# SonSang/dmesh_renderer

Hardware: AMD Instinct MI355X
Metric: fwd+bwd Mpixels/sec @1080p, 500k tris; grad max-abs-err vs ref (higher is better)
Workload: dtype f32

## Files before the change

### dmesh_renderer_amd/build.py

```python
from __future__ import annotations

import os
import shutil
import subprocess
import sys

HERE = os.path.dirname(os.path.abspath(__file__))
CSRC = os.path.join(HERE, "csrc")
LIB = os.path.join(HERE, "libdmesh_renderer_hip.so")
LIB_ABLATION = os.path.join(HERE, "libdmesh_renderer_hip_ablation.so")
SOURCES = ["dmr_api.hip", "dmr_binning.hip", "dmr_tri.hip", "dmr_tet.hip", "dmr_shade.hip", "dmr_texture.hip", "dmr_visibility.hip",
           "dmr_interp.hip"]
HEADERS = ["dmr_device.hpp", "dmr_kernels.hpp", "dmr_placement_key.hpp", "dmr_sort.hpp", "dmr_shade_common.hpp", "dmr_texture_wrap.hpp",
           os.path.join("..", "..", "include", "dmesh_renderer_amd.h"), os.path.join("..", "..", "include", "dmesh_renderer_amd_shade.h"),
           os.path.join("..", "..", "include", "dmesh_renderer_amd_texture.h"),
           os.path.join("..", "..", "include", "dmesh_renderer_amd_visibility.h"),
           os.path.join("..", "..", "include", "dmesh_renderer_amd_deferred.h")]
ARCH = "gfx950"


def _hipcc() -> str:
    for cand in (shutil.which("hipcc"), "/opt/rocm/bin/hipcc"):
        if cand and os.path.exists(cand):
            return cand
    raise RuntimeError("hipcc not found: the HIP extension cannot be built")


def _glue_path() -> str:
    import sysconfig
    return os.path.join(HERE, "_C" + (sysconfig.get_config_var("EXT_SUFFIX") or ".so"))


GLUE_SOURCES = ["dmr_torch.cpp", os.path.join("..", "..", "include", "dmesh_renderer_amd.h"),
                os.path.join("..", "..", "include", "dmesh_renderer_amd_shade.h"),
                os.path.join("..", "..", "include", "dmesh_renderer_amd_texture.h"),
                os.path.join("..", "..", "include", "dmesh_renderer_amd_visibility.h"),
                os.path.join("..", "..", "include", "dmesh_renderer_amd_deferred.h")]


def glue_stale() -> bool:
    out = _glue_path()
    if not os.path.exists(out):
        return True
    t = os.path.getmtime(out)
    return any(os.path.getmtime(os.path.join(CSRC, d)) > t for d in GLUE_SOURCES) or os.path.getmtime(os.path.abspath(__file__)) > t


def build_glue(force: bool = False, verbose: bool = False) -> str:
    out = _glue_path()
    if not force and not glue_stale():
        return out
    import sysconfig
    import torch
    from torch.utils import cpp_extension as ce
    tlib = os.path.join(os.path.dirname(torch.__file__), "lib")
    cxx = shutil.which("g++") or shutil.which("c++")
    if not cxx:
        raise RuntimeError("g++ not found: the PyTorch binding cannot be built")
    cmd = [cxx, "-O2", "-std=c++17", "-fPIC", "-shared", "-D__HIP_PLATFORM_AMD__=1", "-DUSE_ROCM=1", "-DTORCH_EXTENSION_NAME=_C",
           "-DTORCH_API_INCLUDE_EXTENSION_H", f"-D_GLIBCXX_USE_CXX11_ABI={int(torch._C._GLIBCXX_USE_CXX11_ABI)}"]
    cmd += ["-I" + p for p in ce.include_paths()] + ["-I/opt/rocm/include", "-I" + sysconfig.get_paths()["include"]]
    cmd += [os.path.join(CSRC, "dmr_torch.cpp"), "-o", out + ".tmp", "-L" + tlib, "-lc10", "-lc10_hip", "-ltorch_cpu", "-ltorch_hip",
            "-ltorch", "-ltorch_python", "-Wl,-rpath," + tlib, "-ldl"]
    if verbose:
        print(" ".join(cmd), flush=True)
    subprocess.check_call(cmd)
    os.replace(out + ".tmp", out)
    return out


def build_all(force: bool = False, verbose: bool = False):
    res = build(force=force, verbose=verbose), build_glue(force=force, verbose=verbose)
    pkg = sys.modules.get(__package__ or "dmesh_renderer_amd")
    if pkg is not None and type(getattr(pkg, "_C", None)).__name__ == "_NotBuilt":
        import importlib
        pkg._C = importlib.import_module(pkg.__name__ + "._C")
    return res


def stale(lib: str = LIB) -> bool:
    if not os.path.exists(lib):
        return True
    t = os.path.getmtime(lib)
    deps = [os.path.join(CSRC, s) for s in SOURCES + HEADERS] + [os.path.abspath(__file__)]
    return any(os.path.getmtime(d) > t for d in deps)


def build(force: bool = False, verbose: bool = False, ablation: bool = False) -> str:
    lib = LIB_ABLATION if ablation else LIB
    if not force and not stale(lib):
        return lib
    cmd = [_hipcc(), f"--offload-arch={ARCH}", "-O3", "-std=c++17", "-ffp-contract=off", "-fno-slp-vectorize", "-fPIC", "-shared",
           "-Wall", "-Wno-unused-function", "-Wl,-rpath,/opt/rocm/lib", "-o", lib + ".tmp"]
    if ablation:
        cmd.append("-DDMR_ABLATION")
    cmd += [os.path.join(CSRC, s) for s in SOURCES]
    if verbose:
        print(" ".join(cmd), flush=True)
    subprocess.check_call(cmd)
    os.replace(lib + ".tmp", lib)
    return lib


if __name__ == "__main__":
    print(build(force="--force" in sys.argv, verbose=True, ablation="--ablation" in sys.argv))
    if "--ablation" not in sys.argv:
        print(build_glue(force="--force" in sys.argv, verbose=True))
```

### dmesh_renderer_amd/csrc/dmr_api.hip

```cpp
#include <algorithm>
#include <atomic>
#include <chrono>
#include <cstdio>
#include <cstdlib>
#include <cstring>
#include <functional>
#include <map>
#include <mutex>
#include <string>
#include <vector>

#include "dmr_kernels.hpp"
#include "dmr_placement_key.hpp"

namespace {

thread_local std::string g_err;

int fail(const std::string& m) { g_err = m; return 1; }

#define DMR_HIP(expr)                                                                           \
    do {                                                                                        \
        hipError_t e_ = (expr);                                                                 \
        if (e_ != hipSuccess) return fail(std::string(#expr) + ": " + hipGetErrorString(e_));   \
    } while (0)

int caller_output(dmr_alloc_fn alloc, void* ctx, int which, size_t bytes, const char* what, bool idle, hipStream_t st, float** out) {
    *out = nullptr;
    if (bytes == 0) return 0;
    if (!alloc) return fail("null argument");
    float* p = static_cast<float*>(alloc(ctx, which, bytes));
    if (!p) return fail(std::string("allocation of the ") + what + " buffer failed");
    if (idle) DMR_HIP(hipMemsetAsync(p, 0, bytes, st));
    else *out = p;
    return 0;
}

int fragment_k(const dmr_scene* s, int flag, const char* name, const char* macro) {
    const int K = (s->flags & flag) ? DMR_FRAGMENTS_K(s->flags) : 0;
    if ((s->flags & flag) && (K < 1 || K > dmr::FRAG_MAX_K))
        return -fail(std::string(name) + ": K (bits 8-15 of flags, " + macro + ") must be in 1..32, got " + std::to_string(K));
    return K;
}

int fragment_grad_inputs(dmr_alloc_fn alloc, void* ctx, const char* r, const std::string& R, int face_id, int grad_id, size_t npix, int K,
                         const int32_t** face, const float** grad) {
    if (!alloc) return fail("null argument");
    const std::string no = "DMR_FLAG_" + R + "_FRAGMENT_GRADS: no " + r + " fragment ";
    *face = static_cast<const int32_t*>(alloc(ctx, face_id, dmr::FragmentLists::face_bytes(npix, K)));
    if (!*face) return fail(no + "face buffer (DMR_BUF_" + R + "_FRAGMENT_FACES)");
    *grad = static_cast<const float*>(alloc(ctx, grad_id, dmr::FragmentLists::bary_bytes(npix, K)));
    if (!*grad) return fail(no + "bary gradient buffer (DMR_BUF_" + R + "_FRAGMENT_BARY_GRADS)");
    return 0;
}

using dmr::Dims;
using dmr::PointState;
using dmr::FaceState;
using dmr::ImageState;
using dmr::BinningState;
using dmr::Scratch;

constexpr size_t ALIGN = 256;
inline size_t up(size_t n) { return (n + ALIGN - 1) & ~(ALIGN - 1); }

struct Carver {
    char* base; size_t off;
    explicit Carver(void* b) : base(reinterpret_cast<char*>(b)), off(0) {}
    template <class T> T* take(size_t count) {
        T* p = base ? reinterpret_cast<T*>(base + off) : nullptr;
        off += up(count * sizeof(T));
        return p;
    }
};

size_t carve_point(void* b, size_t BP, PointState& s) { Carver c(b); s.vproj = c.take<float4>(BP); return c.off; }
size_t carve_face(void* b, size_t BF, size_t F, size_t T, bool tet, FaceState& s) {
    Carver c(b);
    s.rect = c.take<uint2>(BF); s.key_depth = c.take<float>(BF);
    s.max_depth = tet ? c.take<float>(BF) : nullptr;
    s.tiles_touched = c.take<uint32_t>(BF);
    s.facerec = s.colrec = s.tetrec = nullptr;
    if (tet) {
        s.facerec = c.take<char>(F * dmr::tet_facerec_bytes());
        s.colrec = c.take<char>(F * dmr::tet_colrec_bytes());
        s.tetrec = c.take<char>(T * dmr::tet_tetrec_bytes());
    }
    return c.off;
}
size_t carve_image(void* b, size_t B, size_t ntiles, size_t npix, bool tet, ImageState& s) {
    Carver c(b);
    s.mats = c.take<float>(64 * B);
    s.seed = c.take<int>(1);
    s.mask_offset = c.take<unsigned long long>(2);
    s.tile_count = c.take<uint32_t>(ntiles); s.tile_hits = c.take<uint32_t>(ntiles); s.tile_bound = c.take<uint32_t>(ntiles);
    s.scan_tmp = c.take<uint32_t>(dmr::scan_tmp_words((int)ntiles));
    s.hit_offset = c.take<uint32_t>(ntiles + 1); s.tile_used = c.take<uint32_t>(ntiles); s.hit_total = c.take<unsigned long long>(1);
    s.tile_offset = c.take<uint32_t>(ntiles + 1);
    s.tile_cursor = c.take<uint32_t>(ntiles); s.num_rendered = c.take<int>(1);
    s.tile_order = c.take<uint32_t>(ntiles);
    s.final_T = c.take<float>(npix); s.final_prev_T = c.take<float>(npix); s.n_contrib = c.take<uint32_t>(npix);
    if (tet) {
        s.first_face = c.take<int32_t>(npix); s.first_tet = c.take<int32_t>(npix);
        s.last_face = c.take<int32_t>(npix); s.last_tet = c.take<int32_t>(npix);
        s.is_active = c.take<uint8_t>(npix);
        s.seq = c.take<dmr::TetSeq>(1);
    } else {
        s.first_face = s.first_tet = s.last_face = s.last_tet = nullptr; s.is_active = nullptr;
        s.seq = nullptr;
    }
    return c.off;
}
size_t carve_binning(void* b, size_t R, size_t mask_tiles, size_t seq_tiles, size_t seq_steps, BinningState& s) {
    Carver c(b);
    s.face_list = c.take<uint32_t>(R); s.keys = c.take<uint64_t>(R);
    s.capacity = (uint32_t)std::min<size_t>(R, 0xffffffffu);
    s.mask_offset = c.off;
    s.mask_first = dmr::mask_first_slots(R, mask_tiles);
    if (mask_tiles && R > 0) c.take<uint4>(dmr::mask_slots(R, mask_tiles) * 256);
    s.base = reinterpret_cast<char*>(b); s.seq_offset = c.off; s.seq_steps = (uint32_t)seq_steps;
    if (seq_steps) c.take<char>(dmr::tet_seq_bytes(seq_tiles, seq_steps));
    return c.off;
}

Scratch carve_scratch(const dmr_scene* s, bool tet, const Dims& d, const void* pb, const void* fb, const void* ib,
                      const void* bb = nullptr, size_t R = 0) {
    Scratch c;
    c.point_bytes = carve_point(const_cast<void*>(pb), d.BP, c.ps);
    c.face_bytes = carve_face(const_cast<void*>(fb), d.BF, (size_t)s->F, (size_t)s->T, tet, c.fs);
    c.image_bytes = carve_image(const_cast<void*>(ib), (size_t)s->B, (size_t)d.ntiles, d.npix, tet, c.is);
    carve_binning(const_cast<void*>(bb), R, 0, 0, 0, c.bs);
    return c;
}
dmr_scene canonical(const dmr_scene* s, const float* mats) {
    dmr_scene c = *s;
    const size_t n = 16 * (size_t)s->B;
    c.mv_mats = mats; c.proj_mats = mats + n; c.inv_mv_mats = mats + 2 * n; c.inv_proj_mats = mats + 3 * n;
    c.mats_transposed = 0;
    return c;
}

int check_scene(const dmr_scene* s, bool tet, Dims& d) {
    if (!s) return fail("null scene");
    if (s->B <= 0 || s->W <= 0 || s->H <= 0 || s->P < 0 || s->F < 0 || s->T < 0) return fail("bad dimensions");
    if ((int64_t)s->B * s->P > INT32_MAX || (int64_t)s->B * s->F > INT32_MAX || (int64_t)s->B * s->W * s->H > INT32_MAX)
        return fail("problem too large for 32-bit indexing");
    d.gx = (s->W + dmr::TILE - 1) / dmr::TILE;
    d.gy = (s->H + dmr::TILE - 1) / dmr::TILE;
    if (d.gx > 65535 || d.gy > 65535) return fail("image too large (tile coordinates must fit 16 bits)");
    d.r0 = s->row_begin; d.r1 = s->row_end;
    if (d.r0 == 0 && d.r1 == 0) d.r1 = d.gy;
    d.r0 = std::max(0, std::min(d.gy, d.r0));
    d.r1 = std::max(d.r0, std::min(d.gy, d.r1));
    d.ntiles = s->B * d.gx * d.gy;
    d.BP = (size_t)s->B * s->P; d.BF = (size_t)s->B * s->F; d.npix = (size_t)s->B * s->W * s->H;
    if (tet && s->F > 0 && s->P > 0 && (!s->tets || !s->face_tets || !s->tet_faces)) return fail("tet topology missing");
    if (tet && s->F >= (1 << 28)) return fail("too many faces for the tet renderer (face ids must fit 28 bits)");
    return 0;
}

void* pinned_words() {
    void* p = nullptr;
    if (hipHostMalloc(&p, 64, hipHostMallocCoherent | hipHostMallocPortable) != hipSuccess) return nullptr;
    memset(p, 0, 64);
    return p;
}

struct SizeRead {
    void* slot = nullptr; uint32_t seq = 0;
    volatile unsigned long long* word(int which) const { return reinterpret_cast<volatile unsigned long long*>(slot) + which; }
    uint32_t next_seq() { seq = (seq + 1u) & 0xffffffu; if (seq == 0u) seq = 1u; return seq; }
};
thread_local std::map<int, SizeRead> g_size_read;
int wait_size(volatile unsigned long long* w, uint32_t seq, hipStream_t st, unsigned long long* size) {
    const auto t0 = std::chrono::steady_clock::now();
    for (uint32_t spins = 0;; spins++) {
        const unsigned long long v = *w;
        if ((uint32_t)(v >> 40) == (seq & 0xffffffu)) { std::atomic_thread_fence(std::memory_order_acquire); *size = v & ((1ull << 40) - 1ull); return 0; }
        if ((spins & 1023u) == 1023u && std::chrono::steady_clock::now() - t0 > std::chrono::milliseconds(50)) break;
#if defined(__x86_64__) || defined(__i386__)
        __builtin_ia32_pause();
#endif
    }
    DMR_HIP(hipStreamSynchronize(st));
    const unsigned long long v = *w;
    if ((uint32_t)(v >> 40) != (seq & 0xffffffu)) return fail("the size word was not written (internal error)");
    *size = v & ((1ull << 40) - 1ull);
    return 0;
}

std::mutex g_overflow_mu;
std::map<int, uint32_t*> g_overflow;
uint32_t* overflow_word(int dev, bool create) {
    std::lock_guard<std::mutex> lk(g_overflow_mu);
    auto it = g_overflow.find(dev);
    if (it != g_overflow.end()) return it->second;
    if (!create) return nullptr;
    void* p = pinned_words();
    if (!p) return nullptr;
    return g_overflow[dev] = reinterpret_cast<uint32_t*>(p);
}

bool is_async(const dmr_scene* s, hipStream_t st) {
    if (s->flags & DMR_FLAG_ASYNC) return true;
    hipStreamCaptureStatus cs = hipStreamCaptureStatusNone;
    if (hipStreamIsCapturing(st, &cs) != hipSuccess) { (void)hipGetLastError(); return false; }
    return cs != hipStreamCaptureStatusNone;
}

struct SizeKey {
    int v[7];
    bool operator<(const SizeKey& o) const { return memcmp(v, o.v, sizeof(v)) < 0; }
};
struct SizeGuess { double rendered_per_face = 0.0, hits_per_face = 0.0; uint32_t* seq_steps = nullptr; };
std::mutex g_size_mu;
std::map<SizeKey, SizeGuess> g_size_cache;
std::atomic<uint64_t> g_redo_count{0};
int size_bucket(size_t BF) { int b = 0; while ((BF >> (b + 1)) != 0) b++; return b; }
SizeKey size_key(const dmr_scene* s, bool tet, const Dims& d) {
    return SizeKey{{s->B, s->W, s->H, d.r0, d.r1, tet ? 1 : 0, size_bucket(d.BF)}};
}
double lookup_estimate(const SizeKey& key, double SizeGuess::* field) {
    for (int db : {0, -1, 1}) {
        SizeKey k = key; k.v[6] += db;
        auto it = g_size_cache.find(k);
        if (it != g_size_cache.end() && it->second.*field > 0.0) return it->second.*field;
    }
    return 0.0;
}
uint64_t padded(uint64_t n) { return n + n / 4 + 4096; }

struct Placement { uint32_t* start = nullptr; uint32_t* order = nullptr; int ntiles = 0; uint64_t capacity = 0, built_from = 0; bool valid = false; };
std::mutex g_placement_mu;
std::map<dmr::PlacementKey, Placement> g_placement;
int current_device() { int dev = 0; if (hipGetDevice(&dev) != hipSuccess) { (void)hipGetLastError(); dev = -1; } return dev; }
dmr::PlacementKey placement_key(const SizeKey& key) { return dmr::placement_key(current_device(), key.v, 7); }
uint64_t placement_capacity(uint64_t R, int ntiles) { return R + R / 4 + (uint64_t)dmr::SEG_SLACK * (uint64_t)ntiles; }
bool placement_eligible(bool tet, const Dims& d) { return !tet && d.ntiles <= dmr::SCAN_SINGLE_MAX; }
Placement find_placement(const SizeKey& key, const Dims& d) {
    const dmr::PlacementKey pk = placement_key(key);
    if (pk.device < 0) return Placement{};
    std::lock_guard<std::mutex> lk(g_size_mu);
    auto it = g_placement.find(pk);
    return it != g_placement.end() && it->second.valid && it->second.ntiles == d.ntiles ? it->second : Placement{};
}
void drop_placement(const SizeKey& key) {
    const dmr::PlacementKey pk = placement_key(key);
    std::lock_guard<std::mutex> lk(g_size_mu);
    auto it = g_placement.find(pk);
    if (it != g_placement.end()) it->second.valid = false;
}
int build_placement(const SizeKey& key, const Dims& d, uint64_t R, const ImageState& is, hipStream_t st) {
    const uint64_t capacity = placement_capacity(R, d.ntiles);
    if (capacity > 0x7fffffffu) { drop_placement(key); return 0; }
    const dmr::PlacementKey pk = placement_key(key);
    if (pk.device < 0) return 0;
    std::lock_guard<std::mutex> build_lk(g_placement_mu);
    Placement p;
    {
        std::lock_guard<std::mutex> lk(g_size_mu);
        p = g_placement[pk];
        g_placement[pk].valid = false;
    }
    if (p.start && p.ntiles != d.ntiles) return 0;
    if (!p.start) {
        void* mem = nullptr;
        DMR_HIP(hipMalloc(&mem, sizeof(uint32_t) * (2 * (size_t)d.ntiles + 1)));
        p.start = reinterpret_cast<uint32_t*>(mem); p.order = p.start + d.ntiles + 1; p.ntiles = d.ntiles;
    } else {
        DMR_HIP(hipDeviceSynchronize());
    }
    dmr::launch_build_placement(d.ntiles, is.tile_count, is.tile_order, p.start, p.order, st);
    DMR_HIP(hipStreamSynchronize(st));
    p.capacity = capacity; p.built_from = R; p.valid = true;
    std::lock_guard<std::mutex> lk(g_size_mu);
    g_placement[pk] = p;
    return 0;
}

constexpr uint64_t TET_SEQ_BUDGET = 16ull << 30;
uint64_t march_budget_steps(const Dims& d) {
    return std::max<uint64_t>(TET_SEQ_BUDGET / std::max<uint64_t>(dmr::tet_seq_bytes((size_t)d.ntiles, 4), 1), 1) * 4;
}
uint32_t* march_estimate(const SizeKey& key, const Dims& d, bool create, size_t* seq_steps = nullptr) {
    std::lock_guard<std::mutex> lk(g_size_mu);
    SizeGuess& g = g_size_cache[key];
    if (!g.seq_steps && create && !(g.seq_steps = reinterpret_cast<uint32_t*>(pinned_words()))) (void)hipGetLastError();
    if (seq_steps) {
        const uint64_t longest = g.seq_steps ? *reinterpret_cast<volatile uint32_t*>(g.seq_steps) : 0u;
        *seq_steps = longest ? (size_t)std::min<uint64_t>((longest + longest / 4 + 4 + 3) / 4 * 4, march_budget_steps(d)) : 0;
    }
    return g.seq_steps;
}

using dmr::SizeOut;
using dmr::NOWHERE;

struct Sizing { double SizeGuess::* estimate; uint64_t limit; int word; const char* too_large; const char* no_estimate; };

template <class First, class Then>
int sized(const Sizing& z, const SizeKey& key, size_t BF, bool async, hipStream_t st, uint64_t placed_capacity, uint64_t* size, First first, Then then) {
    int dev = 0;
    DMR_HIP(hipGetDevice(&dev));
    uint32_t* overflow = overflow_word(dev, !async);
    uint64_t guess = placed_capacity;
    if (!placed_capacity) {
        std::lock_guard<std::mutex> lk(g_size_mu);
        const double per_face = lookup_estimate(key, z.estimate);
        if (per_face > 0.0) guess = std::min<uint64_t>(padded((uint64_t)(per_face * (double)BF)), z.limit);
    }
    if (async) {
        if (!guess || !overflow) return fail(z.no_estimate);
        if (first(guess, SizeOut{nullptr, overflow, 0u, (uint32_t)guess})) return 1;
        *size = guess;
        DMR_HIP(hipGetLastError());
        return 0;
    }
    SizeRead& sr = g_size_read[dev];
    if (!sr.slot && !(sr.slot = pinned_words())) return fail("hipHostMalloc failed");
    const uint32_t seq = sr.next_seq();
    if (first(guess, SizeOut{const_cast<unsigned long long*>(sr.word(z.word)), nullptr, seq, 0xffffffffu})) return 1;
    unsigned long long n = 0;
    if (wait_size(sr.word(z.word), seq, st, &n)) return 1;
    const bool full = placed_capacity ? (n & dmr::SIZE_WORD_OVERFLOW) != 0 : n > guess;
    if (placed_capacity) n &= dmr::SIZE_WORD_OVERFLOW - 1ull;
    if (n > z.limit) return fail(z.too_large);
    *size = n;
    if (!guess) {
        if (then(n, false)) return 1;
    } else if (full) {
        g_redo_count.fetch_add(1, std::memory_order_relaxed);
        DMR_HIP(hipStreamSynchronize(st));
        if (then(n, true)) return 1;
    }
    {
        std::lock_guard<std::mutex> lk(g_size_mu);
        g_size_cache[key].*z.estimate = (double)std::max<uint64_t>(n, 1) / (double)std::max<size_t>(BF, 1);
    }
    DMR_HIP(hipGetLastError());
    return 0;
}

int run_forward(const dmr_scene* s, bool tet, const Dims& d, dmr_alloc_fn alloc, void* ctx, hipStream_t st, int* num_rendered,
                const std::function<void(const Scratch&, dmr::ListSize)>& render, size_t min_seq_steps = 0) {
    const Scratch need = carve_scratch(s, tet, d, nullptr, nullptr, nullptr);
    void* pb = alloc(ctx, DMR_BUF_POINT, need.point_bytes);
    void* fb = alloc(ctx, DMR_BUF_FACE, need.face_bytes);
    void* ib = alloc(ctx, DMR_BUF_IMAGE, need.image_bytes);
    if (!pb || !fb || !ib) return fail("scratch allocation failed");
    Scratch c = carve_scratch(s, tet, d, pb, fb, ib);
    const bool async = is_async(s, st);
    const SizeKey key = size_key(s, tet, d);
    size_t seq_steps = 0;
    if (tet) march_estimate(key, d, !async, &seq_steps);
    seq_steps = std::max(seq_steps, min_seq_steps);
    const bool placed = placement_eligible(tet, d);
    const Placement pl = placed ? find_placement(key, d) : Placement{};

    auto front = [&](SizeOut out) {
        dmr::launch_project_verts(*s, d, c, dmr::NO_SEGMENTS, st);
        dmr::launch_setup_faces(*s, d, c, tet, st);
        dmr::launch_scan_tiles(d, c, out, st);
    };
    auto binning = [&](uint64_t capacity) -> int {
        BinningState tb;
        const size_t mask_tiles = tet ? 0 : (size_t)d.ntiles;
        void* bb = alloc(ctx, DMR_BUF_BINNING, carve_binning(nullptr, (size_t)capacity, mask_tiles, (size_t)d.ntiles, seq_steps, tb));
        if (!bb && (capacity > 0 || seq_steps > 0)) return fail("binning allocation failed");
        carve_binning(bb, (size_t)capacity, mask_tiles, (size_t)d.ntiles, seq_steps, c.bs);
        return 0;
    };
    bool exact = false;
    auto rest = [&](uint64_t capacity) -> int {
        if (binning(capacity)) return 1;
        exact = true;
        if (capacity > 0) {
            dmr::launch_scatter_faces(*s, d, c, !tet, st);
            if (!dmr::sorts_own_tiles(d)) dmr::launch_sort_tiles(d, c, st);
        }
        render(c, dmr::NO_LIST_SIZE);
        return 0;
    };
    auto binned = [&](SizeOut out) -> int {
        if (binning(pl.capacity)) return 1;
        dmr::launch_project_verts(*s, d, c, dmr::SegInit{pl.start, pl.order}, st);
        dmr::launch_bin_faces(*s, d, c, st);
        render(c, dmr::ListSize{c.is.num_rendered, out, 1u});
        return 0;
    };

    const Sizing list_entries{&SizeGuess::rendered_per_face, 0x7fffffffu, 0, "num_rendered overflows 31 bits",
                              "asynchronous / captured call without a size estimate: run one default (waiting) call with the same "
                              "view configuration first"};
    uint64_t R = 0;
    int rc = sized(list_entries, key, d.BF, async, st, pl.valid ? pl.capacity : 0, &R,
                   [&](uint64_t guess, SizeOut out) {
                       if (pl.valid) return binned(out);
                       front(out);
                       return guess ? rest(guess) : 0;
                   },
                   [&](uint64_t size, bool redo) { if (redo) front(NOWHERE); return rest(size); });
    *num_rendered = (int)R;
    if (rc == 0 && placed && !async) {
        if (exact) rc = build_placement(key, d, R, c.is, st);
        else if (2 * R < pl.built_from) drop_placement(key);
    }
    return rc;
}

std::atomic<uint32_t> g_prof_mask{0};
struct ProfRec { int stage; hipEvent_t a, b; };
std::mutex g_prof_mu;
std::vector<ProfRec*> g_prof_live, g_prof_free;

}

namespace dmr {
StageScope::StageScope(int stage_, hipStream_t st_) : stage(stage_), st(st_), rec(nullptr) {
    if (!(g_prof_mask.load(std::memory_order_relaxed) & (1u << stage))) return;
    ProfRec* r = nullptr;
    {
        std::lock_guard<std::mutex> lk(g_prof_mu);
        if (!g_prof_free.empty()) { r = g_prof_free.back(); g_prof_free.pop_back(); }
    }
    if (!r) {
        r = new ProfRec();
        if (hipEventCreate(&r->a) != hipSuccess || hipEventCreate(&r->b) != hipSuccess) { delete r; return; }
    }
    r->stage = stage;
    (void)hipEventRecord(r->a, st);
    rec = r;
}
StageScope::~StageScope() {
    if (!rec) return;
    ProfRec* r = reinterpret_cast<ProfRec*>(rec);
    (void)hipEventRecord(r->b, st);
    std::lock_guard<std::mutex> lk(g_prof_mu);
    g_prof_live.push_back(r);
}
int api_fail(const char* m) { return fail(m); }
}

extern "C" {

void dmr_profile_enable(uint32_t mask) { g_prof_mask.store(mask); }

int dmr_profile_collect(double* ms, int64_t* launches) {
    std::vector<ProfRec*> live;
    {
        std::lock_guard<std::mutex> lk(g_prof_mu);
        live.swap(g_prof_live);
    }
    int rc = 0;
    for (ProfRec* r : live) {
        float t = 0.f;
        if (hipEventSynchronize(r->b) != hipSuccess || hipEventElapsedTime(&t, r->a, r->b) != hipSuccess) {
            g_err = "profile event read failed";
            rc = 1;
        } else if (r->stage >= 0 && r->stage < DMR_NUM_STAGES) {
            if (ms) ms[r->stage] += (double)t;
            if (launches) launches[r->stage] += 1;
        }
    }
    std::lock_guard<std::mutex> lk(g_prof_mu);
    for (ProfRec* r : live) g_prof_free.push_back(r);
    return rc;
}

const char* dmr_stage_name(int stage) {
    static const char* names[DMR_NUM_STAGES] = {"k_project_verts", "k_setup_faces", "k_scan_tiles", "k_scatter_faces",
                                                "k_sort_tiles", "k_tri_forward", "k_tri_backward_pix", "k_tri_unpack",
                                                "k_tet_first_intersect", "k_tet_forward", "k_tet_backward",
                                                "k_tri_backward_hits"};
    return (stage >= 0 && stage < DMR_NUM_STAGES) ? names[stage] : "?";
}

const char* dmr_last_error(void) { return g_err.c_str(); }

int dmr_overflowed(int device, int reset) {
    int dev = device;
    if (dev < 0 && hipGetDevice(&dev) != hipSuccess) return 0;
    uint32_t* w = overflow_word(dev, false);
    if (!w) return 0;
    volatile uint32_t* v = w;
    const int r = *v != 0u;
    if (reset) *v = 0u;
    return r;
}
uint64_t dmr_redo_count(void) { return g_redo_count.load(std::memory_order_relaxed); }
int dmr_abi_version(void) { return DMR_ABI_VERSION; }
const char* dmr_build_arch(void) { return "gfx950"; }

int dmr_tri_forward(const dmr_scene* s, float* out_color, float* out_depth, dmr_alloc_fn alloc, void* ctx,
                    void* stream, int* num_rendered) {
    Dims d;
    if (check_scene(s, false, d)) return 1;
    if (!alloc || !num_rendered || !out_color || !out_depth) return fail("null argument");
    *num_rendered = 0;
    const int frag_k = fragment_k(s, DMR_FLAG_TRI_FRAGMENTS, "DMR_FLAG_TRI_FRAGMENTS", "DMR_FRAGMENTS_FLAGS(K)");
    if (frag_k < 0) return 1;
    if (s->P == 0 || s->F == 0) return 0;
    hipStream_t st = reinterpret_cast<hipStream_t>(stream);
    float* fragments = nullptr;
    if (caller_output(alloc, ctx, DMR_BUF_TRI_FRAGMENTS, frag_k ? dmr::FragmentLists::bytes(d.npix, frag_k) : 0, "tri fragment", false, st, &fragments))
        return 1;
    Scratch last{};
    auto render = [&](const Scratch& c, dmr::ListSize size) {
        dmr::launch_tri_forward(canonical(s, c.is.mats), d, c, out_color, out_depth, (s->flags & DMR_FLAG_ALPHA) != 0, size, st);
        last = c;
    };
    if (run_forward(s, false, d, alloc, ctx, st, num_rendered, render)) return 1;
    if (fragments && last.is.n_contrib) {
        dmr::launch_tri_fragments(canonical(s, last.is.mats), d, last, frag_k, fragments, st);
        DMR_HIP(hipGetLastError());
    }
    return 0;
}

int dmr_tri_backward(const dmr_scene* s, const float* dL_dcolor, const float* dL_ddepth, int num_rendered,
                     const void* point_buf, const void* face_buf, const void* binning_buf, const void* image_buf,
                     float* dL_dverts, float* dL_dvcolor, float* dL_dfopacity, float* dL_dvdepth, float* dL_dfintense,
                     dmr_alloc_fn alloc, void* ctx, void* stream) {
    Dims d;
    if (check_scene(s, false, d)) return 1;
    hipStream_t st = reinterpret_cast<hipStream_t>(stream);
    const int frag_k = fragment_k(s, DMR_FLAG_TRI_FRAGMENT_GRADS, "DMR_FLAG_TRI_FRAGMENT_GRADS", "DMR_FRAGMENTS_K");
    if (frag_k < 0) return 1;
    const bool camera = (s->flags & DMR_FLAG_TRI_CAMERA_GRADS) != 0;
    const int grads = camera ? dmr::TRI_GRAD_CAMERA : ((s->flags & DMR_FLAG_TRI_EXACT_GRADS) ? dmr::TRI_GRAD_EXACT : dmr::TRI_GRAD_REF);
    const bool idle = s->P == 0 || s->F == 0 || num_rendered <= 0 || d.r1 <= d.r0;
    float* cam_out = nullptr;
    if (caller_output(alloc, ctx, DMR_BUF_TRI_CAMERA_GRADS, camera ? 128 * (size_t)s->B : 0, "tri camera gradient", idle, st, &cam_out)) return 1;
    const int32_t* frag_face = nullptr;
    const float* frag_grad = nullptr;
    if (frag_k && !idle && fragment_grad_inputs(alloc, ctx, "tri", "TRI", DMR_BUF_TRI_FRAGMENT_FACES, DMR_BUF_TRI_FRAGMENT_BARY_GRADS, d.npix, frag_k, &frag_face, &frag_grad))
        return 1;
    if (idle) {
        if (s->P > 0) {
            DMR_HIP(hipMemsetAsync(dL_dverts, 0, sizeof(float) * 3 * (size_t)s->P, st));
            DMR_HIP(hipMemsetAsync(dL_dvcolor, 0, sizeof(float) * 3 * (size_t)s->P, st));
            DMR_HIP(hipMemsetAsync(dL_dvdepth, 0, sizeof(float) * d.BP, st));
        }
        if (s->F > 0) {
            DMR_HIP(hipMemsetAsync(dL_dfopacity, 0, sizeof(float) * (size_t)s->F, st));
            DMR_HIP(hipMemsetAsync(dL_dfintense, 0, sizeof(float) * d.BF, st));
        }
        if (s->P > 0 && s->F > 0) {
            std::lock_guard<std::mutex> lk(g_size_mu);
            SizeGuess& g = g_size_cache[size_key(s, false, d)];
            if (!(g.hits_per_face > 0.0)) g.hits_per_face = 1.0 / (double)std::max<size_t>(d.BF, 1);
        }
        return 0;
    }
    if (!point_buf || !face_buf || !binning_buf || !image_buf || !alloc) return fail("null scratch buffer");
    const Scratch c = carve_scratch(s, false, d, point_buf, face_buf, image_buf, binning_buf, (size_t)num_rendered);
    const ImageState& is = c.is;

    const size_t vbytes = up(sizeof(float) * dmr::VROW * d.BP), fbytes = up(sizeof(float) * dmr::FROW * d.BF);
    const size_t pbytes = up(sizeof(float4) * 2 * (size_t)d.ntiles * dmr::TILE_PIX);
    const size_t cbytes = camera ? up(sizeof(float) * 32 * (size_t)d.ntiles) : 0;
    auto rest = [&](uint64_t capacity, dmr::HitRegions regions) -> int {
        const size_t hbytes = up(sizeof(dmr::HitRecord) * (size_t)capacity);
        char* work = reinterpret_cast<char*>(alloc(ctx, DMR_BUF_WORK, vbytes + fbytes + cbytes + pbytes + hbytes));
        if (!work) return fail("workspace allocation failed");
        float* vrow = reinterpret_cast<float*>(work);
        float* frow = reinterpret_cast<float*>(work + vbytes);
        float* cam_part = reinterpret_cast<float*>(work + vbytes + fbytes);
        float4* pixrec = reinterpret_cast<float4*>(work + vbytes + fbytes + cbytes);
        dmr::HitRecord* hits = reinterpret_cast<dmr::HitRecord*>(work + vbytes + fbytes + cbytes + pbytes);
        const dmr_scene sc = canonical(s, is.mats);
        dmr::launch_tri_backward_pix(sc, d, c, dL_dcolor, dL_ddepth, pixrec, hits, (uint32_t)capacity, reinterpret_cast<float*>(work),
                                     (vbytes + fbytes + cbytes) / sizeof(float), regions,
                                     (s->flags & DMR_FLAG_ALPHA) != 0, st);
        dmr::launch_tri_backward_hits(sc, d, c, pixrec, hits, (uint32_t)capacity, vrow, frow, grads, camera ? cam_part : nullptr, st);
        if (frag_face)
            dmr::launch_tri_fragment_grads(sc, d, c, frag_k, frag_face, frag_grad, vrow, camera ? cam_part : nullptr, st);
        dmr::launch_tri_unpack(*s, vrow, frow, dL_dverts, dL_dvcolor, dL_dfopacity, dL_dvdepth, dL_dfintense, st);
        if (camera) dmr::launch_camera_reduce(s->B, d.gx * d.gy, 32, cam_part, cam_out, st);
        return 0;
    };
    const dmr::HitRegions scanned{nullptr, nullptr, NOWHERE};
    auto self_laid = [&](SizeOut out) { return dmr::HitRegions{is.hit_offset, is.hit_total, out}; };
    const bool self_regions = d.ntiles <= dmr::SCAN_SINGLE_MAX;
    auto first = [&](uint64_t guess, SizeOut out) -> int {
        if (guess && self_regions) return rest(guess, self_laid(out));
        dmr::launch_scan_hits(d, c, out, st);
        return guess ? rest(guess, scanned) : 0;
    };
    const Sizing hit_records{&SizeGuess::hits_per_face, 0xfffffffeu, 1, "more than 2^32 blended (pixel, face) pairs",
                             "asynchronous / captured call without a size estimate: run one default (waiting) backward with the "
                             "same view configuration first"};
    uint64_t nhits = 0;
    return sized(hit_records, size_key(s, false, d), d.BF, is_async(s, st), st, 0, &nhits, first,
                 [&](uint64_t exact, bool redo) { return rest(exact, redo && self_regions ? self_laid(NOWHERE) : scanned); });
}

int dmr_tet_forward(const dmr_scene* s, float* out_color, float* out_depth, float* out_active, dmr_alloc_fn alloc,
                    void* ctx, void* stream, int* num_rendered) {
    Dims d;
    if (check_scene(s, true, d)) return 1;
    if (!alloc || !num_rendered || !out_color || !out_depth || !out_active) return fail("null argument");
    *num_rendered = 0;
    hipStream_t st = reinterpret_cast<hipStream_t>(stream);
    int frag_k = fragment_k(s, DMR_FLAG_TET_FRAGMENTS, "DMR_FLAG_TET_FRAGMENTS", "DMR_TET_FRAGMENTS_FLAGS(K)");
    if (frag_k < 0) return 1;
    if (s->P == 0 || s->F == 0) frag_k = 0;
    const size_t frag_steps = ((size_t)frag_k + 3) / 4 * 4;
    if (frag_steps > march_budget_steps(d))
        return fail("DMR_FLAG_TET_FRAGMENTS: K = " + std::to_string(frag_k) + " needs a march sequence of " +
                    std::to_string(dmr::tet_seq_bytes((size_t)d.ntiles, frag_steps)) + " bytes (" + std::to_string(frag_steps) +
                    " steps for each of " + std::to_string((size_t)d.ntiles * dmr::TILE_PIX) + " tile pixels), beyond the budget of " +
                    std::to_string(TET_SEQ_BUDGET) + " bytes (16 GiB)");
    float* fragments = nullptr;
    if (caller_output(alloc, ctx, DMR_BUF_TET_FRAGMENTS, frag_k ? dmr::FragmentLists::bytes(d.npix, frag_k) : 0, "tet fragment", false, st, &fragments))
        return 1;
    auto render = [&](const Scratch& c, dmr::ListSize) {
        const dmr_scene sc = canonical(s, c.is.mats);
        dmr::launch_tet_prep(sc, d, c, st);
        dmr::launch_tet_first_intersect(sc, d, c, st);
        dmr::launch_tet_forward(sc, d, c, out_color, out_depth, out_active, (s->flags & DMR_FLAG_ALPHA) != 0, st);
        if (fragments) dmr::launch_tet_fragments(sc, d, c, frag_k, fragments, st);
    };
    return run_forward(s, true, d, alloc, ctx, st, num_rendered, render, frag_steps);
}

int dmr_tet_backward(const dmr_scene* s, const float* dL_dcolor, const float* dL_ddepth, const void* point_buf,
                     const void* face_buf, const void* binning_buf, const void* image_buf, float* dL_dvcolor,
                     float* dL_dfopacity, dmr_alloc_fn alloc, void* ctx, void* stream) {
    Dims d;
    if (check_scene(s, true, d)) return 1;
    hipStream_t st = reinterpret_cast<hipStream_t>(stream);
    const int frag_k = fragment_k(s, DMR_FLAG_TET_FRAGMENT_GRADS, "DMR_FLAG_TET_FRAGMENT_GRADS", "DMR_FRAGMENTS_K");
    if (frag_k < 0) return 1;
    const bool camera = (s->flags & DMR_FLAG_TET_CAMERA_GRADS) != 0;
    const int band_tiles = d.gx * (d.r1 - d.r0);
    float* cam_out = nullptr;
    if (caller_output(alloc, ctx, DMR_BUF_TET_CAMERA_GRADS, camera ? 256 * (size_t)s->B : 0, "tet camera gradient",
                      s->P == 0 || s->F == 0 || band_tiles == 0, st, &cam_out))
        return 1;
    float* full = nullptr;
    const bool full_grads = (s->flags & (DMR_FLAG_TET_FULL_GRADS | DMR_FLAG_TET_CAMERA_GRADS | DMR_FLAG_TET_FRAGMENT_GRADS)) != 0;
    if (caller_output(alloc, ctx, DMR_BUF_TET_GRADS, full_grads ? sizeof(float) * (3 * (size_t)s->P + d.BF) : 0, "tet gradient", false, st, &full))
        return 1;
    if (full) dmr::launch_tet_zero_grads(full, 3 * (int64_t)s->P, full + 3 * (int64_t)s->P, (int64_t)d.BF, st);
    dmr::launch_tet_zero_grads(dL_dvcolor, 3 * (int64_t)s->P, dL_dfopacity, (int64_t)s->F, st);
    if (s->P == 0 || s->F == 0) return 0;
    if (!image_buf || !face_buf) return fail("null scratch buffer");
    const int32_t* frag_face = nullptr;
    const float* frag_grad = nullptr;
    if (frag_k && band_tiles > 0 && fragment_grad_inputs(alloc, ctx, "tet", "TET", DMR_BUF_TET_FRAGMENT_FACES, DMR_BUF_TET_FRAGMENT_BARY_GRADS, d.npix, frag_k, &frag_face, &frag_grad))
        return 1;
    float* cam_part = nullptr;
    if (cam_out) {
        cam_part = static_cast<float*>(alloc(ctx, DMR_BUF_WORK, 256 * (size_t)band_tiles * (size_t)s->B));
        if (!cam_part) return fail("workspace allocation failed");
    }
    const Scratch c = carve_scratch(s, true, d, point_buf, face_buf, image_buf, binning_buf);
    const dmr_scene sc = canonical(s, c.is.mats);
    uint32_t* host_seq_steps = march_estimate(size_key(s, true, d), d, false);
    dmr::launch_tet_backward(sc, d, c, dL_dcolor, dL_ddepth, dL_dvcolor, dL_dfopacity, host_seq_steps, full,
                             full ? full + 3 * (int64_t)s->P : nullptr, cam_part, (s->flags & DMR_FLAG_ALPHA) != 0, st);
    if (frag_face) dmr::launch_tet_fragment_grads(sc, d, c, frag_k, frag_face, frag_grad, full, cam_part, st);
    if (cam_out) dmr::launch_camera_reduce(s->B, band_tiles, 64, cam_part, cam_out, st);
    DMR_HIP(hipGetLastError());
    return 0;
}

namespace {
__global__ void k_invert_mats(const float* __restrict__ in, int count, int transposed, float* __restrict__ out) {
    const int m = blockIdx.x * blockDim.x + threadIdx.x;
    if (m >= count) return;
    double a[16];
#pragma unroll
    for (int k = 0; k < 16; k++) a[k] = (double)in[16 * m + (transposed ? 4 * (k & 3) + (k >> 2) : k)];
    const double s0 = a[0] * a[5] - a[1] * a[4], s1 = a[0] * a[6] - a[2] * a[4], s2 = a[0] * a[7] - a[3] * a[4];
    const double s3 = a[1] * a[6] - a[2] * a[5], s4 = a[1] * a[7] - a[3] * a[5], s5 = a[2] * a[7] - a[3] * a[6];
    const double c5 = a[10] * a[15] - a[11] * a[14], c4 = a[9] * a[15] - a[11] * a[13], c3 = a[9] * a[14] - a[10] * a[13];
    const double c2 = a[8] * a[15] - a[11] * a[12], c1 = a[8] * a[14] - a[10] * a[12], c0 = a[8] * a[13] - a[9] * a[12];
    const double det = s0 * c5 - s1 * c4 + s2 * c3 + s3 * c2 - s4 * c1 + s5 * c0;
    const double r = 1.0 / det;
    double b[16];
    b[0] = (a[5] * c5 - a[6] * c4 + a[7] * c3) * r;   b[1] = (-a[1] * c5 + a[2] * c4 - a[3] * c3) * r;
    b[2] = (a[13] * s5 - a[14] * s4 + a[15] * s3) * r; b[3] = (-a[9] * s5 + a[10] * s4 - a[11] * s3) * r;
    b[4] = (-a[4] * c5 + a[6] * c2 - a[7] * c1) * r;  b[5] = (a[0] * c5 - a[2] * c2 + a[3] * c1) * r;
    b[6] = (-a[12] * s5 + a[14] * s2 - a[15] * s1) * r; b[7] = (a[8] * s5 - a[10] * s2 + a[11] * s1) * r;
    b[8] = (a[4] * c4 - a[5] * c2 + a[7] * c0) * r;   b[9] = (-a[0] * c4 + a[1] * c2 - a[3] * c0) * r;
    b[10] = (a[12] * s4 - a[13] * s2 + a[15] * s0) * r; b[11] = (-a[8] * s4 + a[9] * s2 - a[11] * s0) * r;
    b[12] = (-a[4] * c3 + a[5] * c1 - a[6] * c0) * r; b[13] = (a[0] * c3 - a[1] * c1 + a[2] * c0) * r;
    b[14] = (-a[12] * s3 + a[13] * s1 - a[14] * s0) * r; b[15] = (a[8] * s3 - a[9] * s1 + a[10] * s0) * r;
#pragma unroll
    for (int k = 0; k < 16; k++) out[16 * m + k] = (float)b[k];
}
}

int dmr_invert_mats(const float* in, int count, int transposed, float* out, void* stream) {
    if (count < 0 || (count > 0 && (!in || !out))) return fail("dmr_invert_mats: bad arguments");
    if (count == 0) return 0;
    hipStream_t st = reinterpret_cast<hipStream_t>(stream);
    k_invert_mats<<<dim3((unsigned)((count + 63) / 64)), dim3(64), 0, st>>>(in, count, transposed, out);
    DMR_HIP(hipGetLastError());
    return 0;
}

namespace {
__global__ void k_export_vproj(const float4* v, int64_t n, int what, float* dst) {
    const int64_t i = (int64_t)blockIdx.x * blockDim.x + threadIdx.x;
    if (i >= n) return;
    if (what == 0) { dst[2 * i] = v[i].x; dst[2 * i + 1] = v[i].y; }
    else dst[i] = v[i].z;
}
__global__ void k_export_ranges(const uint32_t* off, const uint32_t* cnt, int64_t n, uint32_t* dst) {
    const int64_t i = (int64_t)blockIdx.x * blockDim.x + threadIdx.x;
    if (i >= n) return;
    const bool empty = cnt[i] == 0;
    dst[2 * i] = empty ? 0u : off[i];
    dst[2 * i + 1] = empty ? 0u : off[i + 1];
}
}

int64_t dmr_export(const dmr_scene* s, int is_tet, int num_rendered, const char* name, const void* point_buf,
                   const void* face_buf, const void* binning_buf, const void* image_buf, void* dst, int64_t cap,
                   void* stream) {
    Dims d;
    if (!name || check_scene(s, is_tet != 0, d)) return -1;
    hipStream_t st = reinterpret_cast<hipStream_t>(stream);
    const Scratch c = carve_scratch(s, is_tet != 0, d, point_buf, face_buf, image_buf, binning_buf, (size_t)std::max(0, num_rendered));
    const FaceState& fs = c.fs; const ImageState& is = c.is;
    const std::string n(name);
    auto plain = [&](const void* src, size_t bytes) -> int64_t {
        if (dst && src && bytes) {
            if (hipMemcpyAsync(dst, src, std::min<size_t>(bytes, (size_t)cap), hipMemcpyDeviceToDevice, st) != hipSuccess) {
                g_err = "export copy failed";
                return -1;
            }
        }
        return (int64_t)bytes;
    };
    if (n == "image" || n == "ndc_z") {
        const size_t bytes = d.BP * (n == "image" ? 8 : 4);
        if (dst && d.BP && (size_t)cap >= bytes)
            k_export_vproj<<<dim3((unsigned)((d.BP + 255) / 256)), dim3(256), 0, st>>>(
                c.ps.vproj, (int64_t)d.BP, n == "image" ? 0 : 1, reinterpret_cast<float*>(dst));
        return (int64_t)bytes;
    }
    if (!is_tet && d.ntiles <= dmr::SCAN_SINGLE_MAX && (n == "ranges" || n == "face_list")) {
        const size_t nt = (size_t)d.ntiles, R = (size_t)std::max(0, num_rendered);
        const size_t bytes = n == "ranges" ? nt * 8 : R * 4;
        if (!dst || (size_t)cap < bytes || bytes == 0) return (int64_t)bytes;
        if (!image_buf || (n == "face_list" && !binning_buf)) { g_err = "null scratch buffer"; return -1; }
        std::vector<uint32_t> off(nt + 1), end(nt), out(bytes / 4, 0u);
        if (hipStreamSynchronize(st) != hipSuccess || hipMemcpy(off.data(), is.tile_offset, 4 * (nt + 1), hipMemcpyDeviceToHost) != hipSuccess ||
            hipMemcpy(end.data(), is.tile_cursor, 4 * nt, hipMemcpyDeviceToHost) != hipSuccess) { g_err = "export copy failed"; return -1; }
        std::vector<uint32_t> lists;
        if (n == "face_list") {
            lists.resize(off[nt]);
            if (off[nt] && hipMemcpy(lists.data(), c.bs.face_list, 4 * (size_t)off[nt], hipMemcpyDeviceToHost) != hipSuccess) { g_err = "export copy failed"; return -1; }
        }
        size_t run = 0;
        for (size_t t = 0; t < nt; t++) {
            const size_t len = dmr::list_end(off.data(), end.data(), (int)t) - off[t];
            if (n == "ranges") { out[2 * t] = len ? (uint32_t)run : 0u; out[2 * t + 1] = len ? (uint32_t)(run + len) : 0u; }
            else for (size_t k = 0; k < len && run + k < R; k++) out[run + k] = lists[off[t] + k];
            run += len;
        }
        if (hipMemcpy(dst, out.data(), bytes, hipMemcpyHostToDevice) != hipSuccess) { g_err = "export copy failed"; return -1; }
        return (int64_t)bytes;
    }
    if (n == "ranges") {
        const size_t bytes = (size_t)d.ntiles * 8;
        if (dst && (size_t)cap >= bytes)
            k_export_ranges<<<dim3((unsigned)((d.ntiles + 255) / 256)), dim3(256), 0, st>>>(
                is.tile_offset, is.tile_count, d.ntiles, reinterpret_cast<uint32_t*>(dst));
        return (int64_t)bytes;
    }
    if (n == "key_depth") return plain(fs.key_depth, d.BF * 4);
    if (n == "max_depth") return is_tet ? plain(fs.max_depth, d.BF * 4) : -1;
    if (n == "tiles_touched") return plain(fs.tiles_touched, d.BF * 4);
    if (n == "face_list") return plain(c.bs.face_list, (size_t)std::max(0, num_rendered) * 4);
    if (n == "final_T") return plain(is.final_T, d.npix * 4);
    if (n == "final_prev_T") return plain(is.final_prev_T, d.npix * 4);
    if (n == "n_contrib") return plain(is.n_contrib, d.npix * 4);
    if (n == "tile_hits") return is_tet ? -1 : plain(is.tile_hits, (size_t)d.ntiles * 4);
    if (is_tet) {
        if (n == "first_face") return plain(is.first_face, d.npix * 4);
        if (n == "first_tet") return plain(is.first_tet, d.npix * 4);
        if (n == "last_face") return plain(is.last_face, d.npix * 4);
        if (n == "last_tet") return plain(is.last_tet, d.npix * 4);
        if (n == "is_active") return plain(is.is_active, d.npix);
        if (n == "tet_seq") return plain(is.seq, 8);
    }
    g_err = "unknown export item: " + n;
    return -1;
}

}
```

Measured before the change: 7805.

## Reorder tile dispatch with host-side block-aware load balancing across XCD classes

After building placement, tile counts and hit counts are copied to the host. A greedy partitioner there assigns 4x4 tile blocks to 8 interleaved classes, which likely correspond to the XCDs, balancing estimated cost. Within each class tiles are sorted longest-first, and the resulting order overwrites the device-built order. The aim is to keep spatially adjacent tiles on the same die for cache locality and to balance per-die work. The cost is host round-trips and synchronisation on the placement build path.

```diff
diff --git a/dmesh_renderer_amd/build.py b/dmesh_renderer_amd/build.py
--- a/dmesh_renderer_amd/build.py
+++ b/dmesh_renderer_amd/build.py
@@ -11,7 +11,7 @@
 LIB_ABLATION = os.path.join(HERE, "libdmesh_renderer_hip_ablation.so")
 SOURCES = ["dmr_api.hip", "dmr_binning.hip", "dmr_tri.hip", "dmr_tet.hip", "dmr_shade.hip", "dmr_texture.hip", "dmr_visibility.hip",
            "dmr_interp.hip"]
-HEADERS = ["dmr_device.hpp", "dmr_kernels.hpp", "dmr_placement_key.hpp", "dmr_sort.hpp", "dmr_shade_common.hpp", "dmr_texture_wrap.hpp",
+HEADERS = ["dmr_device.hpp", "dmr_kernels.hpp", "dmr_placement_key.hpp", "dmr_tile_order.hpp", "dmr_sort.hpp", "dmr_shade_common.hpp", "dmr_texture_wrap.hpp",
            os.path.join("..", "..", "include", "dmesh_renderer_amd.h"), os.path.join("..", "..", "include", "dmesh_renderer_amd_shade.h"),
            os.path.join("..", "..", "include", "dmesh_renderer_amd_texture.h"),
            os.path.join("..", "..", "include", "dmesh_renderer_amd_visibility.h"),
diff --git a/dmesh_renderer_amd/csrc/dmr_api.hip b/dmesh_renderer_amd/csrc/dmr_api.hip
--- a/dmesh_renderer_amd/csrc/dmr_api.hip
+++ b/dmesh_renderer_amd/csrc/dmr_api.hip
@@ -12,6 +12,7 @@
 
 #include "dmr_kernels.hpp"
 #include "dmr_placement_key.hpp"
+#include "dmr_tile_order.hpp"
 
 namespace {
 
@@ -271,6 +272,14 @@
         DMR_HIP(hipDeviceSynchronize());
     }
     dmr::launch_build_placement(d.ntiles, is.tile_count, is.tile_order, p.start, p.order, st);
+    static_assert(dmr::SEG_SLACK >= 1, "a placed call's list capacity covers one entry per tile");
+    const size_t n = (size_t)d.ntiles;
+    std::vector<uint32_t> host(3 * n);
+    DMR_HIP(hipMemcpyAsync(host.data(), is.tile_count, sizeof(uint32_t) * n, hipMemcpyDeviceToHost, st));
+    DMR_HIP(hipMemcpyAsync(host.data() + n, is.tile_hits, sizeof(uint32_t) * n, hipMemcpyDeviceToHost, st));
+    DMR_HIP(hipStreamSynchronize(st));
+    dmr::tile_order(d.ntiles / (d.gx * d.gy), d.gx, d.gy,host.data(), host.data() + n, host.data() + 2 * n);
+    DMR_HIP(hipMemcpyAsync(p.order, host.data() + 2 * n, sizeof(uint32_t) * n, hipMemcpyHostToDevice, st));
     DMR_HIP(hipStreamSynchronize(st));
     p.capacity = capacity; p.built_from = R; p.valid = true;
     std::lock_guard<std::mutex> lk(g_size_mu);
diff --git a/dmesh_renderer_amd/csrc/dmr_tile_order.hpp b/dmesh_renderer_amd/csrc/dmr_tile_order.hpp
--- /dev/null
+++ b/dmesh_renderer_amd/csrc/dmr_tile_order.hpp
@@ -0,0 +1,67 @@
+#pragma once
+
+#include <algorithm>
+#include <cstdint>
+#include <vector>
+
+namespace dmr {
+
+constexpr int ORDER_BLOCK = 4;
+constexpr int ORDER_CLASSES = 8;
+
+inline void tile_order(int B, int gx, int gy, const uint32_t* count, const uint32_t* pairs, uint32_t* order, int block = ORDER_BLOCK) {
+    const int ntiles = B * gx * gy;
+    const int nclass = std::min(ORDER_CLASSES, ntiles);
+    if (ntiles <= 0) return;
+    const int nbx = (gx + block - 1) / block, nby = (gy + block - 1) / block, nblocks = B * nbx * nby;
+    auto block_of = [&](int t) { return ((t / (gx * gy)) * nby + (t / gx) % gy / block) * nbx + t % gx / block; };
+    auto room = [&](int x) { return (ntiles - x + ORDER_CLASSES - 1) / ORDER_CLASSES; };
+
+    std::vector<double> cost((size_t)nblocks, 0.0);
+    for (int t = 0; t < ntiles; t++)
+        if (count[t]) cost[(size_t)block_of(t)] += (double)count[t] + 44.0 + (pairs ? 0.083 * (double)pairs[t] : 0.0);
+    std::vector<int> heavy;
+    for (int k = 0; k < nblocks; k++) if (cost[(size_t)k] > 0.0) heavy.push_back(k);
+    std::stable_sort(heavy.begin(), heavy.end(), [&](int a, int b) { return cost[(size_t)a] > cost[(size_t)b]; });
+    std::vector<int> home((size_t)nblocks, 0);
+    double load[ORDER_CLASSES] = {};
+    for (int k : heavy) {
+        int x = 0;
+        for (int y = 1; y < nclass; y++) if (load[y] < load[x]) x = y;
+        home[(size_t)k] = x; load[x] += cost[(size_t)k];
+    }
+
+    auto longer = [&](uint32_t a, uint32_t b) { return count[a] > count[b]; };
+    std::vector<uint32_t> busy[ORDER_CLASSES], spilled, empty;
+    for (int t = 0; t < ntiles; t++) {
+        if (count[t]) busy[home[(size_t)block_of(t)]].push_back((uint32_t)t);
+        else empty.push_back((uint32_t)t);
+    }
+    for (int x = 0; x < nclass; x++) {
+        std::stable_sort(busy[x].begin(), busy[x].end(), longer);
+        const size_t keep = (size_t)room(x);
+        if (busy[x].size() > keep) {
+            spilled.insert(spilled.end(), busy[x].begin() + (std::ptrdiff_t)keep, busy[x].end());
+            busy[x].resize(keep);
+        }
+    }
+    if (!spilled.empty()) {
+        std::stable_sort(spilled.begin(), spilled.end(), longer);
+        for (uint32_t t : spilled) {
+            int x = -1; size_t most = 0;
+            for (int y = 0; y < nclass; y++) {
+                const size_t left = (size_t)room(y) - busy[y].size();
+                if (left > most) { most = left; x = y; }
+            }
+            busy[x].push_back(t);
+        }
+        for (int x = 0; x < nclass; x++) std::stable_sort(busy[x].begin(), busy[x].end(), longer);
+    }
+    size_t e = 0;
+    for (int x = 0; x < nclass; x++) {
+        const size_t n = (size_t)room(x);
+        for (size_t k = 0; k < n; k++) order[(size_t)x + ORDER_CLASSES * k] = k < busy[x].size() ? busy[x][k] : empty[e++];
+    }
+}
+
+}
```

New measurement: 7955 (median of 6 runs). 1.9% higher.
